# HKUST-KnowComp/DualMessagePassing

Hardware: AMD Instinct MI355X
Metric: (pattern,graph) pairs/sec DMPNN fwd+bwd hid=128 (higher is better)
Workload: dtype f32

## Files before the change

### dualmessagepassing_amd/csrc/dmp_nodechain.hip

```cpp
#include "dmp_mfma_common.h"

namespace dmp {
__device__ int llvm_struct_buffer_load_i32(i32x4 rsrc, int vindex, int voffset, int soffset, int aux) __asm("llvm.amdgcn.struct.buffer.load.i32");
__device__ void llvm_struct_buffer_store_i32(int data, i32x4 rsrc, int vindex, int voffset, int soffset, int aux) __asm("llvm.amdgcn.struct.buffer.store.i32");
namespace {

constexpr int kChainThreads = 512;
constexpr int kChainRows = 128;
constexpr int kChainStrideD = 68;
constexpr int kChainPlane = kChainRows * kChainStrideD;
constexpr int kChainImageBytes = 3 * kChainPlane * 4;
constexpr int kChainPanelBytes = 3 * 128 * 128 * 2;
constexpr int kChainChunkBytes = kChainPanelBytes / 4;
constexpr int kChainLdsBytes = kChainImageBytes + 2 * kChainChunkBytes + kChainRows * 4;
constexpr int kChainMaxPanels = 12;

__device__ __forceinline__ float sbuf_load1(srsrc_t r, int row, uint32_t col_bytes) {
  return __int_as_float(llvm_struct_buffer_load_i32(r, row, (int)col_bytes, 0, 0));
}
__device__ __forceinline__ void sbuf_store1(float v, srsrc_t r, int row, uint32_t col_bytes) {
  llvm_struct_buffer_store_i32(__float_as_int(v), r, row, (int)col_bytes, 0, 0);
}

struct PackArgs {
  const float *W[kChainMaxPanels];
  int64_t ld[kChainMaxPanels];
  int transposed[kChainMaxPanels];
  uint32_t *out;
};
__global__ __launch_bounds__(256) void chain_pack_k(PackArgs p) {
  const int item = (int)blockIdx.x * 256 + (int)threadIdx.x;
  const int lane = item & 63, cb = (item >> 6) & 3, g = item >> 8;
  const int li = lane & 31, h = lane >> 5;
  const float *W = nullptr;
  int64_t ld = 0;
  int tr = 0;
#pragma unroll
  for (int j = 0; j < kChainMaxPanels; ++j)
    if (j == (int)blockIdx.y) { W = p.W[j]; ld = p.ld[j]; tr = p.transposed[j]; }
  const int k0 = 64 * h + 8 * g, c = 32 * cb + li;
  float w[8];
#pragma unroll
  for (int j = 0; j < 8; ++j) w[j] = tr ? W[(int64_t)c * ld + k0 + j] : W[(int64_t)(k0 + j) * ld + c];
  Split8 s;
  split8(make_float4(w[0], w[1], w[2], w[3]), make_float4(w[4], w[5], w[6], w[7]), s);
  uint32_t *o = p.out + (size_t)blockIdx.y * (kChainPanelBytes / 4) + (size_t)g * 3072 + cb * 256 + lane * 4;
  *reinterpret_cast<uint4 *>(o) = make_uint4(s.hi.u[0], s.hi.u[1], s.hi.u[2], s.hi.u[3]);
  *reinterpret_cast<uint4 *>(o + 1024) = make_uint4(s.mid.u[0], s.mid.u[1], s.mid.u[2], s.mid.u[3]);
  *reinterpret_cast<uint4 *>(o + 2048) = make_uint4(s.lo.u[0], s.lo.u[1], s.lo.u[2], s.lo.u[3]);
}

struct ChainArgs {
  const float *A0, *A1, *A2;
  int64_t lda0, lda1, lda2;
  const float *X; int64_t ldx;
  const float *Res; int64_t ldres;
  const float *bias1, *bias2;
  float *O0, *O1, *O2, *O3;
  int64_t ldo0, ldo1, ldo2, ldo3;
  float *partial, *partialA;
  const uint32_t *panels;
  int npanels;
  const int32_t *slot; const int32_t *num_tiles;
  int64_t rows;
  float slope;
};

template <bool BWD, bool FULL>
__global__ __launch_bounds__(kChainThreads) void node_chain_k(ChainArgs p) {
  extern __shared__ __attribute__((aligned(256))) unsigned char lds[];
  uint32_t *Aimg = reinterpret_cast<uint32_t *>(lds);
  unsigned char *Pb = lds + kChainImageBytes;
  int *ids_s = reinterpret_cast<int *>(lds + kChainImageBytes + 2 * kChainChunkBytes);

  const int t = threadIdx.x;
  const int wave = __builtin_amdgcn_readfirstlane(t >> 6);
  const int lane = t & 63, li = lane & 31, h = lane >> 5;
  const int rt = wave >> 1, ch = wave & 1;
  const int q = t & 31, r0 = t >> 5;
  const float slope = __builtin_bit_cast(float, __builtin_amdgcn_readfirstlane(__builtin_bit_cast(int, p.slope)));
  const bool has_res = p.Res != nullptr;
  const int NC = __builtin_amdgcn_readfirstlane(p.npanels) * 4;
  constexpr bool full = FULL;

  const int ntiles = __builtin_amdgcn_readfirstlane(*p.num_tiles);
  const int chunk = (ntiles + (int)gridDim.x - 1) / (int)gridDim.x;
  const int lo = (int)blockIdx.x * chunk;
  const int hi = lo + chunk < ntiles ? lo + chunk : ntiles;
  if (hi <= lo) {
    if (BWD && t < 128) { p.partial[(int64_t)blockIdx.x * 128 + t] = 0.f; p.partialA[(int64_t)blockIdx.x * 128 + t] = 0.f; }
    return;
  }
  const rsrc_t rs_slot = make_rsrc(p.slot, (uint32_t)hi * (kSub * 4u));
  const rsrc_t rs_pan = make_rsrc(p.panels, (uint32_t)NC * (uint32_t)kChainChunkBytes);
  const srsrc_t rs_A0 = make_srsrc(p.A0, p.lda0, p.rows), rs_A1 = make_srsrc(p.A1, p.lda1, p.rows), rs_A2 = make_srsrc(p.A2, p.lda2, p.rows);
  const srsrc_t rs_X = make_srsrc(p.X, p.X ? p.ldx : (int64_t)128, p.X ? p.rows : 0);
  const srsrc_t rs_Res = make_srsrc(p.Res, has_res ? p.ldres : (int64_t)128, has_res ? p.rows : 0);
  const srsrc_t rs_O0 = make_srsrc(p.O0, p.ldo0, p.rows), rs_O1 = make_srsrc(p.O1, p.ldo1, p.rows), rs_O2 = make_srsrc(p.O2, p.ldo2, p.rows);
  const srsrc_t rs_O3 = make_srsrc(p.O3, p.O3 ? p.ldo3 : (int64_t)128, p.O3 ? p.rows : 0);

  int ids[8];
  float4 pre[8];
  auto load_ids = [&](int tile0) {
#pragma unroll
    for (int m = 0; m < 8; ++m) {
      const int idx = tile0 * kSub + r0 + 16 * m;
      const int v = (int)__builtin_amdgcn_raw_buffer_load_b32(rs_slot, idx * 4, 0, 0);
      ids[m] = idx < hi * kSub ? v : -1;
    }
  };
  auto load_rows = [&](srsrc_t rs) {
#pragma unroll
    for (int m = 0; m < 8; ++m) pre[m] = sbuf_load4(rs, ids[m], (uint32_t)q * 16u);
  };
  float4 csA = make_float4(0.f, 0.f, 0.f, 0.f);
  auto stage = [&](bool first) {
#pragma unroll
    for (int m = 0; m < 8; ++m) {
      const int row = r0 + 16 * m;
      if (BWD && first) { csA.x += pre[m].x; csA.y += pre[m].y; csA.z += pre[m].z; csA.w += pre[m].w; }
      uint2 ph, pm, pl;
      split_pair(pre[m].x, pre[m].y, ph.x, pm.x, pl.x);
      split_pair(pre[m].z, pre[m].w, ph.y, pm.y, pl.y);
      uint32_t *d = Aimg + row * kChainStrideD + q * 2;
      *reinterpret_cast<uint2 *>(d) = ph;
      *reinterpret_cast<uint2 *>(d + kChainPlane) = pm;
      *reinterpret_cast<uint2 *>(d + 2 * kChainPlane) = pl;
      if (first && q == 0) ids_s[row] = ids[m];
    }
  };

  f32x16 acc[2];
  auto zero_acc = [&]() {
#pragma unroll
    for (int r = 0; r < 16; ++r) { acc[0][r] = 0.f; acc[1][r] = 0.f; }
  };
  auto product = [&](int pidx) {
#pragma unroll
    for (int cc = 0; cc < 4; ++cc) {
      const int c = 4 * pidx + cc;
      const int nc = c + 1 == NC ? 0 : c + 1;
      uint4 pc[3];
#pragma unroll
      for (int i = 0; i < 3; ++i) {
        const u32x4 v = __builtin_amdgcn_raw_buffer_load_b128(rs_pan, (i * kChainThreads + t) * 16, nc * kChainChunkBytes, 0);
        pc[i] = make_uint4(v.x, v.y, v.z, v.w);
      }
      const unsigned char *pb = Pb + (cc & 1) * kChainChunkBytes;
      const uint32_t *ar = Aimg + (32 * rt + li) * kChainStrideD + 32 * h;
#pragma unroll
      for (int gl = 0; gl < 2; ++gl) {
        const int g = 2 * cc + gl;
        Split8 a;
        a.hi.v = *reinterpret_cast<const bf16x8 *>(ar + 4 * g);
        a.mid.v = *reinterpret_cast<const bf16x8 *>(ar + kChainPlane + 4 * g);
        a.lo.v = *reinterpret_cast<const bf16x8 *>(ar + 2 * kChainPlane + 4 * g);
#pragma unroll
        for (int cbl = 0; cbl < 2; ++cbl) {
          const unsigned char *bq = pb + gl * 12288 + (2 * ch + cbl) * 1024 + lane * 16;
          Split8 b;
          b.hi.v = *reinterpret_cast<const bf16x8 *>(bq);
          b.mid.v = *reinterpret_cast<const bf16x8 *>(bq + 4096);
          b.lo.v = *reinterpret_cast<const bf16x8 *>(bq + 8192);
          acc[cbl] = mfma_x6(a, b, acc[cbl]);
        }
      }
      uint4 *pw = reinterpret_cast<uint4 *>(Pb + ((cc + 1) & 1) * kChainChunkBytes);
#pragma unroll
      for (int i = 0; i < 3; ++i) pw[i * kChainThreads + t] = pc[i];
      lds_barrier();
    }
  };
  int rid[16];
  auto store_acc = [&](srsrc_t rs) {
#pragma unroll
    for (int cb = 0; cb < 2; ++cb)
#pragma unroll
      for (int r = 0; r < 16; ++r) sbuf_store1(acc[cb][r], rs, rid[r], (uint32_t)(64 * ch + 32 * cb + li) * 4u);
  };
  auto acc_to_image = [&]() {
#pragma unroll
    for (int cb = 0; cb < 2; ++cb)
#pragma unroll
      for (int i = 0; i < 8; ++i) {
        const float va = acc[cb][2 * i], vb = acc[cb][2 * i + 1];
        const float got = __shfl_xor((li & 1) ? va : vb, 1, 64);
        const float f0 = (li & 1) ? got : va, f1 = (li & 1) ? vb : got;
        const int r = 2 * i + (li & 1);
        const int row = 32 * rt + (r & 3) + 8 * (r >> 2) + 4 * h;
        uint32_t ph, pm, pl;
        split_pair(f0, f1, ph, pm, pl);
        uint32_t *d = Aimg + row * kChainStrideD + 32 * ch + 16 * cb + (li >> 1);
        d[0] = ph; d[kChainPlane] = pm; d[2 * kChainPlane] = pl;
      }
  };
  float colsum[2] = {0.f, 0.f};

  load_ids(lo);
  load_rows(rs_A0);
  {
    uint4 *pw = reinterpret_cast<uint4 *>(Pb);
#pragma unroll
    for (int i = 0; i < 3; ++i) {
      const u32x4 v = __builtin_amdgcn_raw_buffer_load_b128(rs_pan, (i * kChainThreads + t) * 16, 0, 0);
      pw[i * kChainThreads + t] = make_uint4(v.x, v.y, v.z, v.w);
    }
  }
  for (int g0 = lo; g0 < hi; g0 += 4) {
    stage(true);
    lds_barrier();
#pragma unroll
    for (int qd = 0; qd < 4; ++qd) {
      const int4 v = *reinterpret_cast<const int4 *>(&ids_s[32 * rt + 8 * qd + 4 * h]);
      rid[4 * qd] = v.x; rid[4 * qd + 1] = v.y; rid[4 * qd + 2] = v.z; rid[4 * qd + 3] = v.w;
    }
    if (!BWD) {
      load_rows(rs_A1);
      zero_acc(); product(0); store_acc(rs_O0);
      zero_acc(); product(1); store_acc(rs_O1);
      zero_acc(); product(2);
      stage(false); lds_barrier();
      load_rows(rs_A2);
      product(3);
      stage(false); lds_barrier();
      load_ids(g0 + 4);
      product(4);
      load_rows(rs_A0);
#pragma unroll
      for (int cb = 0; cb < 2; ++cb) {
        const float b = p.bias1[64 * ch + 32 * cb + li];
#pragma unroll
        for (int r = 0; r < 16; ++r) acc[cb][r] = act_fwd(acc[cb][r] + b, slope);
      }
      float res[2][16];
#pragma unroll
      for (int cb = 0; cb < 2; ++cb)
#pragma unroll
        for (int r = 0; r < 16; ++r) res[cb][r] = sbuf_load1(rs_Res, rid[r], (uint32_t)(64 * ch + 32 * cb + li) * 4u);
      store_acc(rs_O2);
      acc_to_image();
      lds_barrier();
      zero_acc(); product(5);
#pragma unroll
      for (int cb = 0; cb < 2; ++cb) {
        const float b = p.bias2[64 * ch + 32 * cb + li];
#pragma unroll
        for (int r = 0; r < 16; ++r) acc[cb][r] = res[cb][r] + (acc[cb][r] + b);
      }
      store_acc(rs_O3);
    } else {
      float hv[2][16];
#pragma unroll
      for (int cb = 0; cb < 2; ++cb)
#pragma unroll
        for (int r = 0; r < 16; ++r) hv[cb][r] = sbuf_load1(rs_X, rid[r], (uint32_t)(64 * ch + 32 * cb + li) * 4u);
      zero_acc(); product(0);
      if (full) load_rows(rs_A1);
      else load_ids(g0 + 4);
#pragma unroll
      for (int cb = 0; cb < 2; ++cb)
#pragma unroll
        for (int r = 0; r < 16; ++r) {
          acc[cb][r] = act_bwd(hv[cb][r], acc[cb][r], slope);
          colsum[cb] += acc[cb][r];
        }
      store_acc(rs_O0);
      acc_to_image();
      lds_barrier();
      zero_acc(); product(1);
      if (!full) load_rows(rs_A0);
      store_acc(rs_O1);
      zero_acc(); product(2); store_acc(rs_O2);
      if (full) {
        zero_acc(); product(3);
        stage(false); lds_barrier();
        load_rows(rs_A2);
        product(4);
        stage(false); lds_barrier();
        load_ids(g0 + 4);
        float res[2][16];
#pragma unroll
        for (int cb = 0; cb < 2; ++cb)
#pragma unroll
          for (int r = 0; r < 16; ++r) res[cb][r] = sbuf_load1(rs_Res, rid[r], (uint32_t)(64 * ch + 32 * cb + li) * 4u);
        product(5);
        load_rows(rs_A0);
#pragma unroll
        for (int cb = 0; cb < 2; ++cb)
#pragma unroll
          for (int r = 0; r < 16; ++r) acc[cb][r] = res[cb][r] + acc[cb][r];
        store_acc(rs_O3);
      }
    }
  }
  if (BWD) {
    float *red = reinterpret_cast<float *>(Pb);
    float *redA = red + 4 * 128;
#pragma unroll
    for (int cb = 0; cb < 2; ++cb) {
      const float s = colsum[cb] + __shfl_xor(colsum[cb], 32, 64);
      if (h == 0) red[rt * 128 + 64 * ch + 32 * cb + li] = s;
    }
    *reinterpret_cast<float4 *>(&redA[r0 * 128 + q * 4]) = csA;
    lds_barrier();
    if (t < 128) {
      float s = red[t];
#pragma unroll
      for (int w = 1; w < 4; ++w) s += red[w * 128 + t];
      p.partial[(int64_t)blockIdx.x * 128 + t] = s;
      float sa = redA[t];
#pragma unroll
      for (int w = 1; w < 16; ++w) sa += redA[w * 128 + t];
      p.partialA[(int64_t)blockIdx.x * 128 + t] = sa;
    }
  }
}

inline unsigned chain_blocks(int64_t tiles_bound) {
  const int64_t want = (tiles_bound + 3) / 4;
  return (unsigned)(want < 1 ? 1 : (want > 256 ? 256 : want));
}

constexpr int kMaxDevicesC = 64;
template <bool BWD, bool FULL>
inline bool chain_lds_ready() {
  static bool done[kMaxDevicesC] = {};
  int dev = 0;
  if (hipGetDevice(&dev) != hipSuccess || dev < 0 || dev >= kMaxDevicesC) dev = 0;
  if (done[dev]) return true;
  const hipError_t e = hipFuncSetAttribute(reinterpret_cast<const void *>(&node_chain_k<BWD, FULL>), hipFuncAttributeMaxDynamicSharedMemorySize, kChainLdsBytes);
  if (e != hipSuccess) { set_last_hip_error(e); return false; }
  done[dev] = true;
  return true;
}

inline bool chain_rows_ok(const float *a, int64_t ld, int64_t rows) {
  return a && ld >= 128 && ld % 4 == 0 && aligned16(a) && stride_ok(ld) && fits4g(rows, ld);
}

}
}

using namespace dmp;

extern "C" {

int64_t dmp_node_chain_blocks(int64_t tiles_bound) { return (int64_t)chain_blocks(tiles_bound); }
int64_t dmp_node_chain_panel_words(void) { return kChainPanelBytes / 4; }

int dmp_node_chain_pack(const dmp_chain_panel *panels, int num_panels, uint32_t *out, void *stream) {
  if (!panels || !out || num_panels < 1 || num_panels > kChainMaxPanels || !aligned16(out)) return DMP_ERR_BAD_ARG;
  PackArgs a{};
  for (int j = 0; j < num_panels; ++j) {
    if (!panels[j].W || panels[j].ld < 128) return DMP_ERR_BAD_ARG;
    a.W[j] = panels[j].W; a.ld[j] = panels[j].ld; a.transposed[j] = panels[j].transposed ? 1 : 0;
  }
  a.out = out;
  chain_pack_k<<<dim3(8, (unsigned)num_panels), 256, 0, (hipStream_t)stream>>>(a);
  return check_launch();
}

int dmp_node_chain_fwd(const float *x, int64_t ldx, const float *S, int64_t lds, const uint32_t *panels, const float *bn, const float *b2,
                       int residual, float slope, const int32_t *slot, const int32_t *num_tiles, int64_t tiles_bound, int64_t rows, int H,
                       float *H1n, int64_t ldh, float *P, int64_t ldp, float *xn, int64_t ldxn, void *stream) {
  if (H != 128 || g_exact_fp32) return DMP_ERR_UNSUPPORTED;
  if (rows < 0 || tiles_bound < 0) return DMP_ERR_BAD_ARG;
  if (!slope_ok(slope)) return DMP_ERR_UNSUPPORTED;
  if (rows == 0 || tiles_bound == 0) return DMP_OK;
  if (!panels || !bn || !b2 || !slot || !num_tiles || !aligned16(panels)) return DMP_ERR_BAD_ARG;
  if (!x || !S || !H1n || !P || !xn || ldx < H || lds < 2 * H || ldh < H || ldp < 2 * H || ldxn < H) return DMP_ERR_BAD_ARG;
  if (!chain_rows_ok(x, ldx, rows) || !chain_rows_ok(S, lds, rows) || !chain_rows_ok(H1n, ldh, rows) || !chain_rows_ok(P, ldp, rows) ||
      !chain_rows_ok(xn, ldxn, rows) || rows >= ((int64_t)1 << 30) || tiles_bound * kSub * 4 >= ((int64_t)1 << 32) - 8192)
    return DMP_ERR_UNSUPPORTED;
  if (!chain_lds_ready<false, true>()) return DMP_ERR_HIP;
  ChainArgs a{};
  a.A0 = x; a.lda0 = ldx; a.A1 = S; a.lda1 = lds; a.A2 = S + H; a.lda2 = lds;
  a.Res = residual ? x : nullptr; a.ldres = ldx; a.bias1 = bn; a.bias2 = b2;
  a.O0 = P; a.ldo0 = ldp; a.O1 = P + H; a.ldo1 = ldp; a.O2 = H1n; a.ldo2 = ldh; a.O3 = xn; a.ldo3 = ldxn;
  a.panels = panels; a.npanels = 6; a.slot = slot; a.num_tiles = num_tiles; a.rows = rows; a.slope = slope;
  node_chain_k<false, true><<<chain_blocks(tiles_bound), kChainThreads, kChainLdsBytes, (hipStream_t)stream>>>(a);
  return check_launch();
}

int dmp_node_chain_bwd(const float *dxn, int64_t ldd, const float *H1n, int64_t ldh, const float *dP, int64_t ldp, const uint32_t *panels,
                       int residual, float slope, const int32_t *slot, const int32_t *num_tiles, int64_t tiles_bound, int64_t rows, int H,
                       float *dPn, int64_t ldn, float *dS, int64_t lds, float *dx, int64_t ldx, float *partial, float *partial_rows,
                       void *stream) {
  if (H != 128 || g_exact_fp32) return DMP_ERR_UNSUPPORTED;
  if (rows < 0 || tiles_bound < 0) return DMP_ERR_BAD_ARG;
  if (!slope_ok(slope)) return DMP_ERR_UNSUPPORTED;
  if (!partial || !partial_rows) return DMP_ERR_BAD_ARG;
  hipStream_t st = (hipStream_t)stream;
  if (rows == 0 || tiles_bound == 0) {
    const size_t bytes = sizeof(float) * 128 * (size_t)chain_blocks(tiles_bound);
    if (hipMemsetAsync(partial, 0, bytes, st) != hipSuccess || hipMemsetAsync(partial_rows, 0, bytes, st) != hipSuccess) return DMP_ERR_HIP;
    return DMP_OK;
  }
  if (!panels || !slot || !num_tiles || !aligned16(panels)) return DMP_ERR_BAD_ARG;
  if (!dxn || !H1n || !dPn || !dS || ldd < H || ldh < H || ldn < H || lds < 2 * H || (dx && (!dP || ldp < 2 * H || ldx < H))) return DMP_ERR_BAD_ARG;
  if (!chain_rows_ok(dxn, ldd, rows) || !chain_rows_ok(H1n, ldh, rows) || !chain_rows_ok(dPn, ldn, rows) || !chain_rows_ok(dS, lds, rows) ||
      (dx && (!chain_rows_ok(dP, ldp, rows) || !chain_rows_ok(dx, ldx, rows))) || rows >= ((int64_t)1 << 30) ||
      tiles_bound * kSub * 4 >= ((int64_t)1 << 32) - 8192)
    return DMP_ERR_UNSUPPORTED;
  if (!(dx ? chain_lds_ready<true, true>() : chain_lds_ready<true, false>())) return DMP_ERR_HIP;
  ChainArgs a{};
  a.A0 = dxn; a.lda0 = ldd;
  a.A1 = dx ? dP : dxn; a.lda1 = dx ? ldp : ldd; a.A2 = dx ? dP + H : dxn; a.lda2 = a.lda1;
  a.X = H1n; a.ldx = ldh; a.Res = (dx && residual) ? dxn : nullptr; a.ldres = ldd;
  a.O0 = dPn; a.ldo0 = ldn; a.O1 = dS; a.ldo1 = lds; a.O2 = dS + H; a.ldo2 = lds; a.O3 = dx; a.ldo3 = ldx;
  a.partial = partial; a.partialA = partial_rows;
  a.panels = panels; a.npanels = dx ? 6 : 3; a.slot = slot; a.num_tiles = num_tiles; a.rows = rows; a.slope = slope;
  if (dx) node_chain_k<true, true><<<chain_blocks(tiles_bound), kChainThreads, kChainLdsBytes, st>>>(a);
  else node_chain_k<true, false><<<chain_blocks(tiles_bound), kChainThreads, kChainLdsBytes, st>>>(a);
  return check_launch();
}

}
```

Before: 489,200.

## Load weight panels directly into LDS and merge paired buffer descriptors

Each panel chunk for the next step is now copied from global memory straight into the alternate LDS buffer with buffer_load_lds. Previously it went through registers and was written to LDS after the MFMA loop; now the code waits on vmcnt before the barrier. Paired halves of the same matrix (S and S+H, P and P+H, dS and dS+H) are now addressed through one descriptor with an soffset of 512 bytes instead of separate descriptors, which reduces scalar register use and argument count. The direct-to-LDS copy saves VGPRs and removes the staging writes, but it relies on wave-to-lane address mapping and on a full vmcnt wait that can also stall on other outstanding loads.

```diff
diff --git a/dualmessagepassing_amd/csrc/dmp_nodechain.hip b/dualmessagepassing_amd/csrc/dmp_nodechain.hip
--- a/dualmessagepassing_amd/csrc/dmp_nodechain.hip
+++ b/dualmessagepassing_amd/csrc/dmp_nodechain.hip
@@ -18,8 +18,8 @@
 __device__ __forceinline__ float sbuf_load1(srsrc_t r, int row, uint32_t col_bytes) {
   return __int_as_float(llvm_struct_buffer_load_i32(r, row, (int)col_bytes, 0, 0));
 }
-__device__ __forceinline__ void sbuf_store1(float v, srsrc_t r, int row, uint32_t col_bytes) {
-  llvm_struct_buffer_store_i32(__float_as_int(v), r, row, (int)col_bytes, 0, 0);
+__device__ __forceinline__ void sbuf_store1(float v, srsrc_t r, int row, uint32_t col_bytes, int block_bytes) {
+  llvm_struct_buffer_store_i32(__float_as_int(v), r, row, (int)col_bytes, block_bytes, 0);
 }
 
 struct PackArgs {
@@ -51,13 +51,13 @@
 }
 
 struct ChainArgs {
-  const float *A0, *A1, *A2;
-  int64_t lda0, lda1, lda2;
+  const float *A0, *A1;
+  int64_t lda0, lda1;
   const float *X; int64_t ldx;
   const float *Res; int64_t ldres;
   const float *bias1, *bias2;
-  float *O0, *O1, *O2, *O3;
-  int64_t ldo0, ldo1, ldo2, ldo3;
+  float *O0, *O1, *O2;
+  int64_t ldo0, ldo1, ldo2;
   float *partial, *partialA;
   const uint32_t *panels;
   int npanels;
@@ -93,11 +93,11 @@
   }
   const rsrc_t rs_slot = make_rsrc(p.slot, (uint32_t)hi * (kSub * 4u));
   const rsrc_t rs_pan = make_rsrc(p.panels, (uint32_t)NC * (uint32_t)kChainChunkBytes);
-  const srsrc_t rs_A0 = make_srsrc(p.A0, p.lda0, p.rows), rs_A1 = make_srsrc(p.A1, p.lda1, p.rows), rs_A2 = make_srsrc(p.A2, p.lda2, p.rows);
+  const srsrc_t rs_A0 = make_srsrc(p.A0, p.lda0, p.rows), rs_A1 = make_srsrc(p.A1, p.lda1, p.rows);
   const srsrc_t rs_X = make_srsrc(p.X, p.X ? p.ldx : (int64_t)128, p.X ? p.rows : 0);
   const srsrc_t rs_Res = make_srsrc(p.Res, has_res ? p.ldres : (int64_t)128, has_res ? p.rows : 0);
-  const srsrc_t rs_O0 = make_srsrc(p.O0, p.ldo0, p.rows), rs_O1 = make_srsrc(p.O1, p.ldo1, p.rows), rs_O2 = make_srsrc(p.O2, p.ldo2, p.rows);
-  const srsrc_t rs_O3 = make_srsrc(p.O3, p.O3 ? p.ldo3 : (int64_t)128, p.O3 ? p.rows : 0);
+  const srsrc_t rs_O0 = make_srsrc(p.O0, p.ldo0, p.rows), rs_O1 = make_srsrc(p.O1, p.ldo1, p.rows);
+  const srsrc_t rs_O2 = make_srsrc(p.O2, p.O2 ? p.ldo2 : (int64_t)128, p.O2 ? p.rows : 0);
 
   int ids[8];
   float4 pre[8];
@@ -109,9 +109,12 @@
       ids[m] = idx < hi * kSub ? v : -1;
     }
   };
-  auto load_rows = [&](srsrc_t rs) {
-#pragma unroll
-    for (int m = 0; m < 8; ++m) pre[m] = sbuf_load4(rs, ids[m], (uint32_t)q * 16u);
+  auto load_rows = [&](srsrc_t rs, int block = 0) {
+#pragma unroll
+    for (int m = 0; m < 8; ++m) {
+      const i32x4 v = llvm_struct_buffer_load_v4i32(rs, ids[m], q * 16, block * 512, 0);
+      pre[m] = make_float4(__int_as_float(v.x), __int_as_float(v.y), __int_as_float(v.z), __int_as_float(v.w));
+    }
   };
   float4 csA = make_float4(0.f, 0.f, 0.f, 0.f);
   auto stage = [&](bool first) {
@@ -140,12 +143,10 @@
     for (int cc = 0; cc < 4; ++cc) {
       const int c = 4 * pidx + cc;
       const int nc = c + 1 == NC ? 0 : c + 1;
-      uint4 pc[3];
-#pragma unroll
-      for (int i = 0; i < 3; ++i) {
-        const u32x4 v = __builtin_amdgcn_raw_buffer_load_b128(rs_pan, (i * kChainThreads + t) * 16, nc * kChainChunkBytes, 0);
-        pc[i] = make_uint4(v.x, v.y, v.z, v.w);
-      }
+#pragma unroll
+      for (int i = 0; i < 3; ++i)
+        __builtin_amdgcn_raw_ptr_buffer_load_lds(rs_pan, (__attribute__((address_space(3))) unsigned char *)(Pb + ((cc + 1) & 1) * kChainChunkBytes + (i * kChainThreads + 64 * wave) * 16),
+                                                 16, (i * kChainThreads + t) * 16, nc * kChainChunkBytes, 0, 0);
       const unsigned char *pb = Pb + (cc & 1) * kChainChunkBytes;
       const uint32_t *ar = Aimg + (32 * rt + li) * kChainStrideD + 32 * h;
 #pragma unroll
@@ -165,18 +166,16 @@
           acc[cbl] = mfma_x6(a, b, acc[cbl]);
         }
       }
-      uint4 *pw = reinterpret_cast<uint4 *>(Pb + ((cc + 1) & 1) * kChainChunkBytes);
-#pragma unroll
-      for (int i = 0; i < 3; ++i) pw[i * kChainThreads + t] = pc[i];
+      asm volatile("s_waitcnt vmcnt(0)" ::: "memory");
       lds_barrier();
     }
   };
   int rid[16];
-  auto store_acc = [&](srsrc_t rs) {
+  auto store_acc = [&](srsrc_t rs, int block = 0) {
 #pragma unroll
     for (int cb = 0; cb < 2; ++cb)
 #pragma unroll
-      for (int r = 0; r < 16; ++r) sbuf_store1(acc[cb][r], rs, rid[r], (uint32_t)(64 * ch + 32 * cb + li) * 4u);
+      for (int r = 0; r < 16; ++r) sbuf_store1(acc[cb][r], rs, rid[r], (uint32_t)(64 * ch + 32 * cb + li) * 4u, block * 512);
   };
   auto acc_to_image = [&]() {
 #pragma unroll
@@ -217,10 +216,10 @@
     if (!BWD) {
       load_rows(rs_A1);
       zero_acc(); product(0); store_acc(rs_O0);
-      zero_acc(); product(1); store_acc(rs_O1);
+      zero_acc(); product(1); store_acc(rs_O0, 1);
       zero_acc(); product(2);
       stage(false); lds_barrier();
-      load_rows(rs_A2);
+      load_rows(rs_A1, 1);
       product(3);
       stage(false); lds_barrier();
       load_ids(g0 + 4);
@@ -237,7 +236,7 @@
       for (int cb = 0; cb < 2; ++cb)
 #pragma unroll
         for (int r = 0; r < 16; ++r) res[cb][r] = sbuf_load1(rs_Res, rid[r], (uint32_t)(64 * ch + 32 * cb + li) * 4u);
-      store_acc(rs_O2);
+      store_acc(rs_O1);
       acc_to_image();
       lds_barrier();
       zero_acc(); product(5);
@@ -247,7 +246,7 @@
 #pragma unroll
         for (int r = 0; r < 16; ++r) acc[cb][r] = res[cb][r] + (acc[cb][r] + b);
       }
-      store_acc(rs_O3);
+      store_acc(rs_O2);
     } else {
       float hv[2][16];
 #pragma unroll
@@ -264,17 +263,17 @@
           acc[cb][r] = act_bwd(hv[cb][r], acc[cb][r], slope);
           colsum[cb] += acc[cb][r];
         }
-      store_acc(rs_O0);
+      store_acc(rs_O1);
       acc_to_image();
       lds_barrier();
       zero_acc(); product(1);
       if (!full) load_rows(rs_A0);
-      store_acc(rs_O1);
-      zero_acc(); product(2); store_acc(rs_O2);
+      store_acc(rs_O0);
+      zero_acc(); product(2); store_acc(rs_O0, 1);
       if (full) {
         zero_acc(); product(3);
         stage(false); lds_barrier();
-        load_rows(rs_A2);
+        load_rows(rs_A1, 1);
         product(4);
         stage(false); lds_barrier();
         load_ids(g0 + 4);
@@ -289,7 +288,7 @@
         for (int cb = 0; cb < 2; ++cb)
 #pragma unroll
           for (int r = 0; r < 16; ++r) acc[cb][r] = res[cb][r] + acc[cb][r];
-        store_acc(rs_O3);
+        store_acc(rs_O2);
       }
     }
   }
@@ -374,9 +373,9 @@
     return DMP_ERR_UNSUPPORTED;
   if (!chain_lds_ready<false, true>()) return DMP_ERR_HIP;
   ChainArgs a{};
-  a.A0 = x; a.lda0 = ldx; a.A1 = S; a.lda1 = lds; a.A2 = S + H; a.lda2 = lds;
+  a.A0 = x; a.lda0 = ldx; a.A1 = S; a.lda1 = lds;
   a.Res = residual ? x : nullptr; a.ldres = ldx; a.bias1 = bn; a.bias2 = b2;
-  a.O0 = P; a.ldo0 = ldp; a.O1 = P + H; a.ldo1 = ldp; a.O2 = H1n; a.ldo2 = ldh; a.O3 = xn; a.ldo3 = ldxn;
+  a.O0 = P; a.ldo0 = ldp; a.O1 = H1n; a.ldo1 = ldh; a.O2 = xn; a.ldo2 = ldxn;
   a.panels = panels; a.npanels = 6; a.slot = slot; a.num_tiles = num_tiles; a.rows = rows; a.slope = slope;
   node_chain_k<false, true><<<chain_blocks(tiles_bound), kChainThreads, kChainLdsBytes, (hipStream_t)stream>>>(a);
   return check_launch();
@@ -405,9 +404,9 @@
   if (!(dx ? chain_lds_ready<true, true>() : chain_lds_ready<true, false>())) return DMP_ERR_HIP;
   ChainArgs a{};
   a.A0 = dxn; a.lda0 = ldd;
-  a.A1 = dx ? dP : dxn; a.lda1 = dx ? ldp : ldd; a.A2 = dx ? dP + H : dxn; a.lda2 = a.lda1;
+  a.A1 = dx ? dP : dxn; a.lda1 = dx ? ldp : ldd;
   a.X = H1n; a.ldx = ldh; a.Res = (dx && residual) ? dxn : nullptr; a.ldres = ldd;
-  a.O0 = dPn; a.ldo0 = ldn; a.O1 = dS; a.ldo1 = lds; a.O2 = dS + H; a.ldo2 = lds; a.O3 = dx; a.ldo3 = ldx;
+  a.O0 = dS; a.ldo0 = lds; a.O1 = dPn; a.ldo1 = ldn; a.O2 = dx; a.ldo2 = ldx;
   a.partial = partial; a.partialA = partial_rows;
   a.panels = panels; a.npanels = dx ? 6 : 3; a.slot = slot; a.num_tiles = num_tiles; a.rows = rows; a.slope = slope;
   if (dx) node_chain_k<true, true><<<chain_blocks(tiles_bound), kChainThreads, kChainLdsBytes, st>>>(a);
```

Measured after the change: 491,300 (median of 6 runs). No clear change (+0.4%).
